# nlapier2/Metalign

Measured on AMD Instinct MI355X. Metric: 150bp reads/s end-to-end (CMash filter + profile), higher is better.
Workload: dtype u64; 1 GPU; configs[2]: 10M reads vs 10k-genome DB, multi-k {21,31,51} containment — 10000000 synthetic 150bp reads/GPU vs 10000-genome sketch DB (50000 bp genomes, n=1000), k in [21, 31, 51], 12498882 alignment records/GPU, 10001 taxa, 1 MI355X per rank; inputs resident in HBM; stage_a_definition=reference_pipeline, hash_mode=0, stage_a_match=kmer

## Files before the change

include/metalign_hip.h:

```cpp
#ifndef METALIGN_HIP_H
#define METALIGN_HIP_H

#include <stdint.h>

#ifdef __cplusplus
extern "C" {
#endif

#define MG_ABI_VERSION 1

typedef enum mg_status {
  MG_OK = 0,
  MG_ERR_HIP = -1,
  MG_ERR_ARG = -2,
  MG_ERR_CAPACITY = -3,
  MG_ERR_STATE = -4,
  MG_ERR_NOMEM = -5
} mg_status;

#define MG_MAX_K 64

typedef struct mg_aln_rec {
  uint32_t ref_new;
  uint32_t matched;
// ... 240 lines not shown
uint64_t mg_refdb_ngenomes(const mg_refdb* db);
uint64_t mg_refdb_max_hash(const mg_refdb* db);
const mg_db* mg_refdb_kmax_table(const mg_refdb* db);
void mg_refdb_free(mg_refdb* db);
int mg_refpipe_containment_dev(const mg_sketch* q, const mg_refdb* db, uint32_t ci, uint32_t* const* d_hits,
                               uint32_t* const* d_sizes);
int mg_refpipe_mark_dev(const mg_sketch* q, const mg_refdb* db, uint32_t ci, uint32_t* d_hits_kmax, uint32_t* d_sizes_kmax);
int mg_refpipe_count_dev(const mg_refdb* db, const uint32_t* const* d_marks, uint32_t* const* d_hits,
                         uint32_t* const* d_sizes);
int mg_refdb_marks(const mg_refdb* db, int ki, uint32_t** d_marks, uint64_t* nwords);

typedef struct mg_kcounts mg_kcounts;
int mg_refdb_index_kmers(mg_refdb* db, const uint64_t* kmer_hi, const uint64_t* kmer_lo);
int mg_refdb_has_kmer_index(const mg_refdb* db);
uint64_t mg_refdb_distinct_kmers(const mg_refdb* db);
int mg_refdb_kmer_heads(const mg_refdb* db, uint32_t* head);
int mg_kcounts_new(const mg_refdb* db, mg_kcounts** out);
int mg_kcounts_reset(mg_kcounts* kc);
int mg_count_kmers_dev(const uint8_t* d_bases, const uint64_t* d_offsets, uint64_t nreads, uint64_t nbases, const mg_refdb* db,
                       mg_kcounts* kc);
int mg_kcounts_stats(const mg_kcounts* kc, uint64_t* out4);
int mg_kcounts_download(const mg_kcounts* kc, const mg_refdb* db, uint32_t* per_pair);
int mg_kcounts_device(const mg_kcounts* kc, uint32_t** d_counts, uint64_t* n);
int mg_kcounts_wait(const mg_kcounts* kc);
uint64_t mg_kcounts_pack2_bytes(const mg_kcounts* kc);
int mg_kcounts_pack2_dev(const mg_kcounts* kc, uint32_t* d_out);
int mg_kcounts_merge2_dev(mg_kcounts* kc, const uint32_t* d_all, uint32_t nranks, uint64_t stride_dwords);
void mg_kcounts_free(mg_kcounts* kc);
int mg_refpipe_mark_counts_dev(const mg_kcounts* kc, const mg_refdb* db, uint32_t ci, uint32_t* d_hits_kmax, uint32_t* d_sizes_kmax);
int mg_refpipe_mark_counts_ptr_dev(const uint32_t* d_counts, const mg_refdb* db, uint32_t ci, uint32_t* d_hits_kmax,
                                   uint32_t* d_sizes_kmax);
int mg_refpipe_containment_counts_dev(const mg_kcounts* kc, const mg_refdb* db, uint32_t ci, uint32_t* const* d_hits,
                                      uint32_t* const* d_sizes);
int mg_refdb_set_count_share(const mg_refdb* db, uint32_t rank, uint32_t world);

typedef struct mg_profile mg_profile;

int mg_profile_begin_dev(const mg_aln_rec* d_recs, uint64_t nrecs,
                         int has_lookahead, const uint32_t* d_ref2tax,
                         uint32_t nref, uint32_t ntax, double pct_id,
                         mg_profile** out);
int mg_profile_acc_reset(uint64_t* d_count, uint64_t* d_bases, uint64_t* d_first_seen,
                         uint64_t* d_scalars, uint32_t ntax);
int mg_profile_map_launch(mg_profile* p);
int mg_profile_state_map(const mg_profile* p, uint8_t map[2]);
int mg_profile_map_words_dev(mg_profile* p, int64_t* d_out3);
// ... 158 lines not shown
```

metalign_amd/_hip.py:

```python
import ctypes
import os

import numpy as np

_HERE = os.path.dirname(os.path.abspath(__file__))
LIB_PATH = os.environ.get("MG_LIB_PATH") or os.path.join(_HERE, "libmetalign_hip.so")

REC_DTYPE = np.dtype([("ref_new", "<u4"), ("matched", "<u4"), ("total", "<u4"), ("flag_len", "<u4")])
NEW_BIT = 0x80000000
REF_MASK = 0x7FFFFFFF
LEN_SHIFT = 12
MAX_SEQLEN = (1 << 20) - 1
U64_MAX = 0xFFFFFFFFFFFFFFFF
MAX_K = 64

EXPORTS = [
    "mg_abi_version", "mg_debug_set", "mg_debug_get", "mg_device_count", "mg_init", "mg_init_on_stream", "mg_shutdown", "mg_last_error",
    "mg_device_name", "mg_mem_info", "mg_mem_trim", "mg_dev_malloc", "mg_dev_free", "mg_memcpy_h2d", "mg_memcpy_d2h", "mg_dev_memset", "mg_sync",
    "mg_host_alloc", "mg_host_free", "mg_memcpy_d2h_async", "mg_memcpy_h2d_async",
    "mg_event_create", "mg_event_record", "mg_event_synchronize", "mg_event_destroy", "mg_stage_c_side_stream", "mg_stage_a_side_stream", "mg_stage_a_workgroups_per_cu", "mg_stage_c_join",
    "mg_prof_enable", "mg_prof_only", "mg_prof_reset", "mg_prof_get",
    "mg_refdb_index_kmers", "mg_refdb_has_kmer_index", "mg_refdb_distinct_kmers", "mg_refdb_kmer_heads", "mg_kcounts_new", "mg_kcounts_reset", "mg_count_kmers_dev",
    "mg_kcounts_stats", "mg_kcounts_download", "mg_kcounts_device", "mg_kcounts_wait", "mg_kcounts_pack2_bytes", "mg_kcounts_pack2_dev", "mg_kcounts_merge2_dev", "mg_kcounts_free", "mg_refpipe_mark_counts_dev", "mg_refpipe_mark_counts_ptr_dev",
    "mg_refpipe_containment_counts_dev", "mg_refdb_set_count_share",
    "mg_set_count_saturation", "mg_count_saturation", "mg_set_hash_mode", "mg_hash_mode", "mg_hash_mode1_ks", "mg_sketch_reads_dev", "mg_sketch_reads_dev_async", "mg_sketch_reads_multi_dev_async", "mg_sketch_resolve", "mg_filter_build", "mg_filter_download", "mg_filter_from_bits", "mg_filter_log2_bits", "mg_filter_make_resident", "mg_filter_drop_resident", "mg_filter_use_resident", "mg_filter_resident_bytes", "mg_filter_free",
    "mg_sketch_reads_filtered_dev", "mg_sketch_reads_filtered_dev_async", "mg_sketch_from_pairs_dev", "mg_sketch_merge_dev", "mg_sketch_merge_dev_async", "mg_sketch_split", "mg_sketch_slice_words_dev", "mg_sketch_set_bound", "mg_sketch_size", "mg_sketch_truncated", "mg_sketch_last_hash",
    "mg_sketch_kmers_seen", "mg_sketch_device_ptrs", "mg_sketch_download", "mg_sketch_free", "mg_sketch_reads",
    "mg_sketch_stream_begin", "mg_sketch_stream_begin_counts", "mg_sketch_stream_add_dev", "mg_sketch_stream_add_file", "mg_sketch_stream_finish", "mg_sketch_stream_nreads", "mg_sketch_stream_nbases", "mg_sketch_stream_free",
    "mg_reads_parse_dev", "mg_reads_parse_prefix_dev", "mg_reads_parse", "mg_reads_parse_bam_prefix_dev", "mg_reads_from_bam_file", "mg_reads_count", "mg_reads_nbases", "mg_reads_device_ptrs",
    "mg_reads_download", "mg_reads_free",
    "mg_genomes_parse_dev", "mg_genomes_count", "mg_genomes_nbases", "mg_genomes_device_ptrs", "mg_genomes_download", "mg_genomes_free",
    "mg_genomes_stream_open", "mg_genomes_stream_next", "mg_genomes_stream_stats", "mg_genomes_stream_close",
    "mg_sketch_genomes_dev", "mg_sketch_genomes_prefix_dev", "mg_sketch_genomes_kmers_dev",
    "mg_acc_index_build", "mg_acc_index_free", "mg_sam_tokenize_dev", "mg_sam_tokenize", "mg_paf_tokenize_dev", "mg_paf_tokenize", "mg_sam_stream_file", "mg_bam_stream_file", "mg_bam_tokenize_dev", "mg_sam_batch_count",
    "mg_sam_batch_last_qname", "mg_sam_batch_device_ptr", "mg_sam_batch_download", "mg_sam_batch_free",
    "mg_sam_tokenize_keyed_dev", "mg_bam_tokenize_keyed_dev", "mg_sam_batch_keys_download", "mg_collate_order_dev", "mg_sam_batch_collate_dev",
    "mg_sam_stream_file_collated", "mg_bam_stream_file_collated",
    "mg_sam_tokenize_named_dev", "mg_sam_tokenize_named", "mg_bam_tokenize_named_dev", "mg_sam_stream_file_named", "mg_bam_stream_file_named",
    "mg_sam_batch_names_size", "mg_sam_batch_names_download", "mg_profile_commit_assign_dev",
    "mg_sam_tokenize_dev_ex", "mg_sam_tokenize_ex", "mg_bam_tokenize_dev_ex", "mg_sam_stream_file_ex", "mg_bam_stream_file_ex",
    "mg_sam_batch_places_download", "mg_sam_batch_places_device_ptr",
    "mg_coverage_create", "mg_coverage_add_dev", "mg_coverage_result", "mg_coverage_free",
    "mg_depth_create", "mg_depth_add_dev", "mg_depth_finish", "mg_depth_fetch_rows", "mg_depth_fetch_windows", "mg_depth_free",
    "mg_sam_batch_edits_download", "mg_sam_batch_edits_device_ptr",
    "mg_identity_create", "mg_identity_add_dev", "mg_identity_result", "mg_identity_fetch_hist", "mg_identity_free",
    "mg_sam_batch_bases_download", "mg_sam_batch_bases_device_ptr",
# ... 729 lines not shown
    def add_reads(self, reads):
        p_b, p_o = reads.device_ptrs()
        self.add_dev(p_b, p_o, reads.count, reads.nbases)

    def stats(self):
        out = np.zeros(12, np.uint64)
        self.hip._chk(self.hip.lib.mg_kcounts_stats(self.handle, _np(out, ctypes.c_uint64)))
        st = dict(kmers=int(out[0]), runs=int(out[1]), passed=int(out[2]), matches=int(out[3]))
        if out[6]:
            st.update(clk_drain=int(out[4]) * 64, clk_hits=int(out[5]) * 64, clk_kernel=int(out[6]) * 64, entries_looked_at=int(out[7]),
                      windows_scanned=int(out[8]), longest_lane_windows=int(out[9]), longest_lane_entries=int(out[10]), drains=int(out[11]))
        return st

    def download(self):
        npairs = self.table.sizes()[0]
        out = np.zeros(max(npairs, 1), np.uint32)
        self.hip._chk(self.hip.lib.mg_kcounts_download(self.handle, self.table.handle, _np(out, ctypes.c_uint32)))
        return out[:npairs]

    def device(self):
        p, n = _vp(), ctypes.c_uint64(0)
        self.hip._chk(self.hip.lib.mg_kcounts_device(self.handle, ctypes.byref(p), ctypes.byref(n)))
        return int(p.value or 0), int(n.value)

    def wait(self):
        self.hip._chk(self.hip.lib.mg_kcounts_wait(self.handle))

    def pack2_bytes(self):
        self.hip.lib.mg_kcounts_pack2_bytes.restype = ctypes.c_uint64
        return int(self.hip.lib.mg_kcounts_pack2_bytes(self.handle))

    def pack2_dev(self, d_out):
        self.hip._chk(self.hip.lib.mg_kcounts_pack2_dev(self.handle, ctypes.c_void_p(int(d_out))))

    def merge2_dev(self, d_all, nranks, stride_bytes):
        self.hip._chk(self.hip.lib.mg_kcounts_merge2_dev(self.handle, ctypes.c_void_p(int(d_all)), ctypes.c_uint32(int(nranks)),
                                                         ctypes.c_uint64(int(stride_bytes) // 4)))

    def free(self):
        if self.handle:
            self.hip.lib.mg_kcounts_free(self.handle)
            self.handle = None

    def __del__(self):
        try:
            self.free()
# ... 1316 lines not shown
```

metalign_amd/csrc/mg_contain.hip:

```cpp
#include <memory>

#include "mg_internal.h"

namespace mg {

constexpr int kMaxSmallK = 3;
struct ContainK {
  const uint64_t* q;
  const uint32_t* qc;
  uint64_t qn, q_last;
  const uint64_t* meta;
  uint32_t* idx;
  unsigned shift;
  uint64_t idx_buckets;
  uint32_t build_index;
  const uint64_t* ph;
  const uint32_t* pg;
  const uint32_t* gsize;
  uint64_t npairs, ngenomes;
  uint64_t tile0;
  uint32_t* hits_part;
  uint32_t* sizes_part;
  uint32_t* hits;
  uint32_t* sizes;
  const uint32_t* head;
// ... 290 lines not shown
      p[j] = 0xffffffffu; g[j] = 0;
      if (i < K.n) { p[j] = cid[i]; g[j] = cgen[i]; }
    }
    uint32_t w[kPer];
#pragma unroll
    for (int j = 0; j < kPer; ++j) w[j] = p[j] != 0xffffffffu ? marks[p[j] >> 5] : 0u;
#pragma unroll
    for (int j = 0; j < kPer; ++j)
      if ((w[j] >> (p[j] & 31u)) & 1u) atomicAdd(&hits[g[j]], 1u);
  }
}

__global__ void k_refpipe_reduce(const CountArgs a) {
  const uint64_t g0 = (uint64_t)blockIdx.x * blockDim.x + threadIdx.x;
  const uint64_t stride = (uint64_t)gridDim.x * blockDim.x;
  for (int ki = 0; ki < a.nk; ++ki) {
    const CountK& K = a.k[ki];
    for (uint64_t g = g0; g < K.ngenomes; g += stride) {
      uint32_t h = 0;
      for (uint32_t c = 0; c < a.copies; ++c) h += K.hits_part[(uint64_t)c * K.ngenomes + g];
      K.hits[g] = h;
      K.sizes[g] = K.gsize[g];
    }
  }
}

__global__ void k_iota_u32(uint32_t* v, uint64_t n) {
  uint64_t i = (uint64_t)blockIdx.x * blockDim.x + threadIdx.x;
  const uint64_t stride = (uint64_t)gridDim.x * blockDim.x;
  for (; i < n; i += stride) v[i] = (uint32_t)i;
}

__global__ void k_pair_genomes(const uint32_t* __restrict__ orig, uint64_t n, const uint64_t* __restrict__ offsets,
                               uint64_t ngenomes, uint32_t* __restrict__ pair_gen) {
  uint64_t i = (uint64_t)blockIdx.x * blockDim.x + threadIdx.x;
  const uint64_t stride = (uint64_t)gridDim.x * blockDim.x;
  for (; i < n; i += stride) {
    const uint64_t o = orig[i];
    uint64_t lo = 0, hi = ngenomes;
    while (hi - lo > 1) {
      const uint64_t mid = (lo + hi) >> 1;
      if (offsets[mid] <= o) lo = mid; else hi = mid;
    }
    pair_gen[i] = (uint32_t)lo;
  }
}
// ... 351 lines not shown
    K.cid = rp->small[s].cid.as<uint32_t>() + lo;
    K.cgen = rp->small[s].cgen.as<uint32_t>() + lo;
    K.n = hi - lo;
    K.tile0 = tiles;
    tiles += (K.n + kCTile - 1) / kCTile;
    K.ngenomes = G;
    K.marks = d_marks ? d_marks[s] : rp->marks.as<uint32_t>() + rp->small[s].marks_at;
    K.gsize = rp->small[s].gsize.as<uint32_t>();
    K.hits_part = d_part + (uint64_t)s * copies * G;
    K.hits = d_hits[s];
    K.sizes = d_sizes[s];
  }
  a.ntiles = tiles;
  ProfScope ps("refpipe_count");
  if (!prezeroed)
    hipLaunchKernelGGL(k_zero_u32, dim3(grid_for((uint64_t)m * copies * G, 256, (unsigned)c.num_cus * 8)), dim3(256), 0, st, d_part,
                       (uint64_t)m * copies * G);
  if (tiles) hipLaunchKernelGGL(k_refpipe_count, dim3(grid_cap(grid_for(tiles, 1, (unsigned)c.num_cus * 8), "kb_grid")), dim3(kCT), 0, st, a);
  hipLaunchKernelGGL(k_refpipe_reduce, dim3(grid_for(G, 256, (unsigned)c.num_cus * 4)), dim3(256), 0, st, a);
  MG_HIP(hipGetLastError());
  return MG_OK;
}

extern "C" {

int mg_containment_multi_dev(int nk, const mg_sketch* const* qs, const mg_db* const* dbs, uint32_t ci, uint32_t* const* d_hits,
                             uint32_t* const* d_sizes) {
  return containment_launch(nk, qs, dbs, ci, d_hits, d_sizes, nullptr);
}

int mg_refpipe_mark_dev(const mg_sketch* q, const mg_refdb* db, uint32_t ci, uint32_t* d_hits_kmax, uint32_t* d_sizes_kmax) {
  if (!q || !db) return fail(MG_ERR_ARG, "null argument");
  MG_TRY(refdb_ready(db));
  const mg_db* kdb = &db->kmax;
  return containment_launch(1, &q, &kdb, ci, &d_hits_kmax, &d_sizes_kmax, db);
}

int mg_refdb_set_count_share(const mg_refdb* db, uint32_t rank, uint32_t world) {
  if (!db || world == 0 || rank >= world) return fail(MG_ERR_ARG, "rank %u of %u", rank, world);
  db->share_rank = rank;
  db->share_world = world;
  return MG_OK;
}

int mg_refpipe_count_dev(const mg_refdb* db, const uint32_t* const* d_marks, uint32_t* const* d_hits, uint32_t* const* d_sizes) {
  MG_REQUIRE_READY();
// ... 13 lines not shown
  MG_REQUIRE_READY();
  if (!kc || !db || !d_hits_kmax || !d_sizes_kmax) return fail(MG_ERR_ARG, "null argument");
  MG_TRY(refdb_ready(db));
  if (!db->kidx) return fail(MG_ERR_STATE, "the table has no k-mer index (mg_refdb_index_kmers)");
  uint32_t* d_counts = nullptr;
  uint64_t n = 0;
  MG_TRY(mg_kcounts_device(kc, &d_counts, &n));
  if (n != db->kmax.total) return fail(MG_ERR_ARG, "these counters belong to another table");
  MG_TRY(kcounts_wait(kc));
  return match_launch(d_counts, db, ci, d_hits_kmax, d_sizes_kmax);
}

int mg_refpipe_mark_counts_ptr_dev(const uint32_t* d_counts, const mg_refdb* db, uint32_t ci, uint32_t* d_hits_kmax, uint32_t* d_sizes_kmax) {
  MG_REQUIRE_READY();
  if (!d_counts || !db || !d_hits_kmax || !d_sizes_kmax) return fail(MG_ERR_ARG, "null argument");
  MG_TRY(refdb_ready(db));
  if (!db->kidx) return fail(MG_ERR_STATE, "the table has no k-mer index (mg_refdb_index_kmers)");
  return match_launch(d_counts, db, ci, d_hits_kmax, d_sizes_kmax);
}

int mg_refpipe_containment_counts_dev(const mg_kcounts* kc, const mg_refdb* db, uint32_t ci, uint32_t* const* d_hits, uint32_t* const* d_sizes) {
  if (!kc || !db || !d_hits || !d_sizes) return fail(MG_ERR_ARG, "null argument");
  const int last = db->nk - 1;
  MG_TRY(mg_refpipe_mark_counts_dev(kc, db, ci, d_hits[last], d_sizes[last]));
  return refpipe_count_launch(db, nullptr, d_hits, d_sizes);
}

int mg_containment_dev(const mg_sketch* q, const mg_db* db, uint32_t ci, uint32_t* d_hits, uint32_t* d_sizes) {
  return mg_containment_multi_dev(1, &q, &db, ci, &d_hits, &d_sizes);
}

int mg_containment(const uint64_t* q_hashes, const uint32_t* q_counts, uint64_t qn, int q_truncated, uint32_t ci,
                   const uint64_t* db_hashes, const uint64_t* db_offsets, uint64_t ngenomes, uint32_t* out_hits,
                   uint32_t* out_sizes) {
  MG_REQUIRE_READY();
  std::unique_ptr<mg_sketch> sk(new mg_sketch());
  MG_TRY(sk->hashes.alloc(qn * sizeof(uint64_t)));
  MG_TRY(sk->counts.alloc(qn * sizeof(uint32_t)));
  MG_TRY(mg_memcpy_h2d(sk->hashes.p, q_hashes, qn * sizeof(uint64_t)));
  MG_TRY(mg_memcpy_h2d(sk->counts.p, q_counts, qn * sizeof(uint32_t)));
  sk->n = qn;
  sk->truncated = q_truncated;
  sk->last_hash = qn ? q_hashes[qn - 1] : 0;
  mg_db* db = nullptr;
  MG_TRY(mg_db_upload(db_hashes, db_offsets, ngenomes, &db));
  std::unique_ptr<mg_db> dbg(db);
// ... 11 lines not shown
```

metalign_amd/csrc/mg_core.hip:

```cpp
#include <cstring>

#include "mg_internal.h"

namespace mg {

static thread_local char g_err[512] = "";

Context& ctx() {
  static Context c;
  return c;
}

int fail(int code, const char* fmt, ...) {
  va_list ap;
  va_start(ap, fmt);
  vsnprintf(g_err, sizeof(g_err), fmt, ap);
  va_end(ap);
  return code;
}

static const char* const kDebugKeys[] = {
    "k3_hashed", "k3_flush_tiles", "k3_grid", "lds_pad", "force_list", "distinct_hint_ppm", "resident_scan", "no_fused", "resident_ablate",
    "flush_order", "no_avx2", "gzip_threads", "pgzip_chunk", "pgzip_thp", "pgzip_timing", "stream_thin", "stream_threads", "inflate_trace", "inflate_loose_find", "shares_threads", "kc_wg_per_cu", "kc_ablate", "kc_stagger", "kc_gate_extra", "inflate_dev_max_bytes", "kc_grid", "k1_grid", "kb_grid", "collate_defer", "genome_slab_bytes", "genome_guard", "cov_grid", "depth_grid", "mm_hash_bits", "ident_grid", "var_grid"};
static int64_t g_debug[sizeof(kDebugKeys) / sizeof(kDebugKeys[0])] = {};
static int debug_index(const char* key) {
  for (size_t i = 0; i < sizeof(kDebugKeys) / sizeof(kDebugKeys[0]); ++i)
    if (strcmp(kDebugKeys[i], key) == 0) return (int)i;
  return -1;
}
int64_t dbg(const char* key) {
  const int i = debug_index(key);
  return i < 0 ? 0 : g_debug[i];
}

static uint64_t size_class(uint64_t n) {
  if (n < 256) return 256;
  uint64_t p = 256;
  while (p < n) {
    if (p + p / 2 >= n) return p + p / 2;
    p <<= 1;
  }
  return p;
}

static void seal_open_batch();
static void release_completed_batches();
// ... 509 lines not shown
```

metalign_amd/csrc/mg_internal.h:

```cpp
#pragma once
#include <hip/hip_runtime.h>

#include <cstdarg>
#include <cstdlib>
#include <cstdint>
#include <cstdio>
#include <map>
#include <memory>
#include <string>
#include <utility>
#include <vector>

#include "../../include/metalign_hip.h"

namespace mg {

constexpr uint64_t kReservedHash = 0xFFFFFFFFFFFFFFFFull;

struct ProfEntry {
  uint64_t launches = 0;
  double total_ms = 0.0;
};

struct DevBuf;
// ... 321 lines not shown
struct mg_db {
  mg::DevBuf pair_hash;
  mg::DevBuf pair_gen;
  mg::DevBuf gsize;
  mg::DevBuf offsets;
  uint64_t ngenomes = 0;
  uint64_t total = 0;
  uint64_t max_hash = 0;
};

namespace mg {
struct KmerIndex {
  int k = 0;
  uint64_t ndistinct = 0, nentries = 0, nbuckets = 0;
  uint32_t gbits = 0;
  uint64_t gate_words = 0;
  uint32_t bmask = 0;
  DevBuf gate;
  DevBuf shared;
  DevBuf prim;
  DevBuf ovf;
  uint64_t novf = 0;
  DevBuf head;
};
int kcounts_wait(const mg_kcounts* kc);
}

struct mg_refdb {
  mg_db kmax;
  int nk = 0;
  int ks[4] = {0, 0, 0, 0};
  mg::DevBuf kmer_hi, kmer_lo;
  struct Small {
    mg::DevBuf pa, pb;
    mg::DevBuf cid, cgen;
    mg::DevBuf gsize;
    uint64_t nprefix = 0, ncount = 0;
    uint64_t marks_at = 0, marks_n = 0;
  } small[3];
  mg::DevBuf marks;
  uint64_t marks_words = 0;
  mutable uint32_t* count_part = nullptr;
  mutable uint32_t count_copies = 0;
  mutable uint64_t count_gen = 0;
  mutable mg::UploadJob* pending = nullptr;
  mutable bool unchecked = false;
  mutable uint32_t share_rank = 0, share_world = 1;
  mutable int failed = 0;
  std::unique_ptr<mg::KmerIndex> kidx;
  ~mg_refdb();
};
namespace mg { int refdb_ready(const mg_refdb* db); int check_pairs_dev(const mg_db& db); }
```

metalign_amd/csrc/mg_kcount.hip:

```cpp
#include <algorithm>
#include <memory>

#include "mg_internal.h"
#include "mg_kcount_core.h"
#include "mg_sketch_dev.h"

namespace mg {

namespace {

inline unsigned g256(uint64_t n) { return grid_for(n ? n : 1, 256, (unsigned)ctx().num_cus * 8); }
#define KC_FOR(i, n) for (uint64_t i = (uint64_t)blockIdx.x * blockDim.x + threadIdx.x; i < (n); i += (uint64_t)gridDim.x * blockDim.x)

__global__ void k_kc_canon(const uint64_t* __restrict__ khi, const uint64_t* __restrict__ klo, uint64_t n, int k,
                           uint64_t* __restrict__ chi, uint64_t* __restrict__ clo, uint32_t* __restrict__ iota) {
  KC_FOR(i, n) {
    const KcWin c = kc_canonical(kc_from_right(khi[i], klo[i], k), k);
    chi[i] = ((uint64_t)c.w[0] << 32) | c.w[1];
    clo[i] = ((uint64_t)c.w[2] << 32) | c.w[3];
    iota[i] = (uint32_t)i;
  }
}
__global__ void k_kc_gather(const uint64_t* __restrict__ src, const uint32_t* __restrict__ idx, uint64_t n, uint64_t* __restrict__ dst) {
  KC_FOR(i, n) dst[i] = src[idx[i]];
// ... 11 lines not shown
    const KcWin x{{(uint32_t)(hi[j] >> 32), (uint32_t)hi[j], (uint32_t)(lo[j] >> 32), (uint32_t)lo[j]}};
    dhi[id] = hi[j];
    dlo[id] = lo[j];
    dhead[id] = order[j];
    uint32_t keys[kKcMaxCands];
    nkeys[id] = (uint32_t)kc_table_keys(x, k, keys);
  }
}
__global__ void k_kc_emit_keys(const uint64_t* __restrict__ dhi, const uint64_t* __restrict__ dlo, const uint64_t* __restrict__ kbefore,
                               uint64_t nd, int k, uint32_t bmask, uint64_t* __restrict__ ekey, uint32_t* __restrict__ eid) {
  KC_FOR(id, nd) {
    const KcWin x{{(uint32_t)(dhi[id] >> 32), (uint32_t)dhi[id], (uint32_t)(dlo[id] >> 32), (uint32_t)dlo[id]}};
    uint32_t keys[kKcMaxCands];
    const int n = kc_table_keys(x, k, keys);
    for (int t = 0; t < n; ++t) {
      ekey[kbefore[id] + (uint64_t)t] = ((uint64_t)(keys[t] & bmask) << 32) | keys[t];
      eid[kbefore[id] + (uint64_t)t] = (uint32_t)id;
    }
  }
}
__global__ void k_kc_pair_heads(const uint32_t* __restrict__ order, const uint32_t* __restrict__ flag, const uint64_t* __restrict__ before,
                                const uint32_t* __restrict__ dhead, uint64_t n, uint32_t* __restrict__ head) {
  KC_FOR(j, n) head[order[j]] = dhead[before[j] + flag[j] - 1];
}
__global__ void k_kc_entries(const uint64_t* __restrict__ skey, const uint32_t* __restrict__ perm, const uint64_t* __restrict__ dhi,
                             const uint64_t* __restrict__ dlo, const uint32_t* __restrict__ dhead, uint64_t nd, int k, uint32_t gshift,
                             KcEntry* __restrict__ ent, uint32_t* __restrict__ gate, uint32_t* __restrict__ shared) {
  KC_FOR(j, nd) {
    const uint32_t id = perm[j];
    const uint64_t h = dhi[id], l = dlo[id];
    KcEntry e;
    e.w[0] = (uint32_t)(h >> 32); e.w[1] = (uint32_t)h; e.w[2] = (uint32_t)(l >> 32); e.w[3] = (uint32_t)l;
    e.head = dhead[id];
    e.key = (uint32_t)skey[j];
    e.off = kc_table_key_offset(KcWin{{e.w[0], e.w[1], e.w[2], e.w[3]}}, k, e.key);
    e.pad = 0;
    ent[j] = e;
    if (j == 0 || skey[j - 1] != skey[j]) {
      const uint32_t g = e.key >> gshift, bit = 1u << (g & 31u);
      if (atomicOr(&gate[g >> 5], bit) & bit) atomicOr(&shared[g >> 5], bit);
    }
  }
}
__global__ void k_kc_offsets(const uint64_t* __restrict__ skey, uint64_t nd, uint64_t nb, uint32_t* __restrict__ offs) {
  KC_FOR(j, nd + 1) {
    const uint64_t first = j == 0 ? 0 : (skey[j - 1] >> 32) + 1;
// ... 547 lines not shown
int kcounts_order(const mg_kcounts* kc, hipStream_t st) {
  if (kc && kc->ev && kc->ev_stream && kc->ev_stream != st) MG_HIP(hipStreamWaitEvent(st, kc->ev, 0));
  return MG_OK;
}
int kcounts_wait(const mg_kcounts* kc) { return kcounts_order(kc, ctx().stream); }
static int kcounts_wrote(mg_kcounts* kc, hipStream_t st) {
  MG_HIP(hipEventRecord(kc->ev, st));
  kc->ev_stream = st;
  return MG_OK;
}
static hipStream_t kcounts_stage_stream() {
  Context& c = ctx();
  return c.a_side ? (c.a_side == 2 ? c.stream_a2 : c.stream_a) : c.stream;
}

__global__ void k_kc_copy_words(const uint32_t* __restrict__ src, uint32_t* __restrict__ dst, uint64_t nwords) {
  const uint64_t n4 = nwords / 4;
  const uint4* __restrict__ s4 = reinterpret_cast<const uint4*>(src);
  uint4* __restrict__ d4 = reinterpret_cast<uint4*>(dst);
  KC_FOR(i, n4) d4[i] = s4[i];
  KC_FOR(i, nwords - 4 * n4) dst[4 * n4 + i] = src[4 * n4 + i];
}

__global__ void k_kc_pack2(const uint32_t* __restrict__ counts, uint64_t n, uint32_t* __restrict__ out) {
  KC_FOR(w, (n + 15) / 16) {
    uint32_t v = 0;
#pragma unroll
    for (int j = 0; j < 16; ++j) {
      const uint64_t i = w * 16 + (uint64_t)j;
      const uint32_t c = i < n ? counts[i] : 0u;
      v |= (c > 3u ? 3u : c) << (2 * j);
    }
    out[w] = v;
  }
}
__global__ void k_kc_merge2(const uint32_t* __restrict__ all, uint32_t nranks, uint64_t stride, uint64_t n, uint32_t* __restrict__ counts) {
  KC_FOR(w, (n + 15) / 16) {
    uint32_t s[16];
#pragma unroll
    for (int j = 0; j < 16; ++j) s[j] = 0;
    for (uint32_t r = 0; r < nranks; ++r) {
      const uint32_t v = all[(uint64_t)r * stride + w];
#pragma unroll
      for (int j = 0; j < 16; ++j) s[j] += (v >> (2 * j)) & 3u;
    }
#pragma unroll
// ... 31 lines not shown
  DevBuf chi, clo, iota, ord1, ord2, s_lo, s_hi, g_hi, flag, before, dhi, dlo, dhead, nkeys, kbefore, ekey, eid, skey, perm;
  uint64_t nd = 0, ne = 0;
  if (n) {
    MG_TRY(chi.alloc(n * 8)); MG_TRY(clo.alloc(n * 8)); MG_TRY(iota.alloc(n * 4)); MG_TRY(ord1.alloc(n * 4)); MG_TRY(ord2.alloc(n * 4));
    MG_TRY(s_lo.alloc(n * 8)); MG_TRY(s_hi.alloc(n * 8)); MG_TRY(g_hi.alloc(n * 8)); MG_TRY(flag.alloc(n * 4)); MG_TRY(before.alloc((n + 2) * 8));
    hipLaunchKernelGGL(k_kc_canon, dim3(g256(n)), dim3(256), 0, st, db->kmer_hi.as<uint64_t>(), db->kmer_lo.as<uint64_t>(), n, k,
                       chi.as<uint64_t>(), clo.as<uint64_t>(), iota.as<uint32_t>());
    MG_TRY(sort_pairs(clo.as<uint64_t>(), s_lo.as<uint64_t>(), iota.as<uint32_t>(), ord1.as<uint32_t>(), n));
    hipLaunchKernelGGL(k_kc_gather, dim3(g256(n)), dim3(256), 0, st, chi.as<uint64_t>(), ord1.as<uint32_t>(), n, g_hi.as<uint64_t>());
    MG_TRY(sort_pairs(g_hi.as<uint64_t>(), s_hi.as<uint64_t>(), ord1.as<uint32_t>(), ord2.as<uint32_t>(), n));
    hipLaunchKernelGGL(k_kc_gather, dim3(g256(n)), dim3(256), 0, st, clo.as<uint64_t>(), ord2.as<uint32_t>(), n, s_lo.as<uint64_t>());
    hipLaunchKernelGGL(k_kc_heads, dim3(g256(n)), dim3(256), 0, st, s_hi.as<uint64_t>(), s_lo.as<uint64_t>(), n, flag.as<uint32_t>());
    MG_HIP(hipGetLastError());
    MG_TRY(exclusive_sum_u32_to_u64(flag.as<uint32_t>(), before.as<uint64_t>(), n, &nd));
    MG_TRY(dhi.alloc(nd * 8)); MG_TRY(dlo.alloc(nd * 8)); MG_TRY(dhead.alloc(nd * 4)); MG_TRY(nkeys.alloc((nd + 1) * 4));
    MG_TRY(kbefore.alloc((nd + 2) * 8));
    hipLaunchKernelGGL(k_kc_distinct, dim3(g256(n)), dim3(256), 0, st, s_hi.as<uint64_t>(), s_lo.as<uint64_t>(), ord2.as<uint32_t>(),
                       flag.as<uint32_t>(), before.as<uint64_t>(), n, k, dhi.as<uint64_t>(), dlo.as<uint64_t>(), dhead.as<uint32_t>(),
                       nkeys.as<uint32_t>());
    hipLaunchKernelGGL(k_kc_pair_heads, dim3(g256(n)), dim3(256), 0, st, ord2.as<uint32_t>(), flag.as<uint32_t>(), before.as<uint64_t>(),
                       dhead.as<uint32_t>(), n, ix->head.as<uint32_t>());
    MG_HIP(hipGetLastError());
  }
  ix->ndistinct = nd;
  unsigned bb = 8;
  while (bb < 28 && (1ull << bb) < nd) ++bb;
  ix->bmask = (1u << bb) - 1u;
  ix->nbuckets = 1ull << bb;
  const int64_t gx = dbg("kc_gate_extra");
  ix->gbits = kc_gate_bits(nd, gx > 0 ? (uint32_t)gx : kKcGateExtra);
  ix->gate_words = (1ull << ix->gbits) / 32 + 2;
  MG_TRY(ix->gate.alloc(ix->gate_words * 4));
  MG_TRY(ix->shared.alloc(ix->gate_words * 4));
  MG_HIP(hipMemsetAsync(ix->gate.p, 0, ix->gate_words * 4, st));
  MG_HIP(hipMemsetAsync(ix->shared.p, 0, ix->gate_words * 4, st));
  if (nd) {
    MG_TRY(exclusive_sum_u32_to_u64(nkeys.as<uint32_t>(), kbefore.as<uint64_t>(), nd, &ne));
    MG_TRY(ekey.alloc((ne + 1) * 8)); MG_TRY(eid.alloc((ne + 1) * 4)); MG_TRY(skey.alloc((ne + 1) * 8)); MG_TRY(perm.alloc((ne + 1) * 4));
    hipLaunchKernelGGL(k_kc_emit_keys, dim3(g256(nd)), dim3(256), 0, st, dhi.as<uint64_t>(), dlo.as<uint64_t>(), kbefore.as<uint64_t>(), nd, k,
                       ix->bmask, ekey.as<uint64_t>(), eid.as<uint32_t>());
    MG_HIP(hipGetLastError());
    MG_TRY(sort_pairs(ekey.as<uint64_t>(), skey.as<uint64_t>(), eid.as<uint32_t>(), perm.as<uint32_t>(), ne));
  }
  ix->nentries = ne;
  DevBuf offs, ent, extra, obefore;
  MG_TRY(offs.alloc((ix->nbuckets + 2) * 4));
// ... 39 lines not shown
  if (!db->kidx) return fail(MG_ERR_STATE, "the table has no k-mer index (mg_refdb_index_kmers)");
  std::unique_ptr<mg_kcounts> kc(new mg_kcounts());
  kc->n = db->kmax.total;
  kc->live_words = db->kidx->gate_words;
  kc->sat_words = kKcSlots * db->kidx->nbuckets + db->kidx->novf + 4;
  kc->gate = db->kidx->gate.p;
  MG_TRY(kc->counts.alloc((kc->n + 1) * 4));
  MG_TRY(kc->live.alloc(kc->live_words * 4));
  MG_TRY(kc->sat.alloc(kc->sat_words * 4));
  MG_TRY(kc->stats.alloc(12 * 8));
  MG_HIP(hipEventCreateWithFlags(&kc->ev, hipEventDisableTiming));
  MG_TRY(mg_kcounts_reset(kc.get()));
  *out = kc.release();
  return MG_OK;
}

int mg_kcounts_reset(mg_kcounts* kc) {
  MG_REQUIRE_READY();
  if (!kc) return fail(MG_ERR_ARG, "null argument");
  Context& c = ctx();
  if (!c.stream_r) MG_HIP(hipStreamCreateWithFlags(&c.stream_r, hipStreamNonBlocking));
  hipStream_t st = c.stream_r;
  MG_TRY(kcounts_order(kc, st));
  hipLaunchKernelGGL(k_kc_copy_words, dim3(g256(kc->live_words / 4 + 1)), dim3(256), 0, st, static_cast<const uint32_t*>(kc->gate),
                     kc->live.as<uint32_t>(), kc->live_words);
  MG_HIP(hipGetLastError());
  kc->epoch = kc->epoch % 255u + 1u;
  if (kc->epoch == 1u) MG_HIP(hipMemsetAsync(kc->sat.p, 0, kc->sat_words * 4, st));
  MG_HIP(hipMemsetAsync(kc->counts.p, 0, (kc->n + 1) * 4, st));
  MG_HIP(hipMemsetAsync(kc->stats.p, 0, 12 * 8, st));
  return kcounts_wrote(kc, st);
}

int mg_kcounts_wait(const mg_kcounts* kc) {
  MG_REQUIRE_READY();
  if (!kc) return fail(MG_ERR_ARG, "null argument");
  return kcounts_wait(kc);
}

uint64_t mg_kcounts_pack2_bytes(const mg_kcounts* kc) { return kc ? ((kc->n + 15) / 16) * 4 : 0; }

int mg_kcounts_pack2_dev(const mg_kcounts* kc, uint32_t* d_out) {
  MG_REQUIRE_READY();
  if (!kc || !d_out) return fail(MG_ERR_ARG, "null argument");
  if (ctx().count_sat == 0 || ctx().count_sat > 3)
    return fail(MG_ERR_STATE, "two bits hold a counter that saturates at 3 or below (it saturates at %u): exchange the counters themselves", ctx().count_sat);
  MG_TRY(kcounts_wait(kc));
  if (kc->n) hipLaunchKernelGGL(k_kc_pack2, dim3(g256((kc->n + 15) / 16)), dim3(256), 0, ctx().stream, kc->counts.as<uint32_t>(), kc->n, d_out);
  MG_HIP(hipGetLastError());
  return MG_OK;
}

int mg_kcounts_merge2_dev(mg_kcounts* kc, const uint32_t* d_all, uint32_t nranks, uint64_t stride_dwords) {
// ... 56 lines not shown
}

int mg_kcounts_download(const mg_kcounts* kc, const mg_refdb* db, uint32_t* per_pair) {
  MG_REQUIRE_READY();
  if (!kc || !db || !db->kidx || !per_pair) return fail(MG_ERR_ARG, "null argument");
  if (kc->n != db->kmax.total) return fail(MG_ERR_ARG, "these counters belong to another table");
  if (!kc->n) return MG_OK;
  MG_TRY(kcounts_wait(kc));
  DevBuf out;
  MG_TRY(out.alloc(kc->n * 4));
  hipLaunchKernelGGL(k_kc_per_pair, dim3(g256(kc->n)), dim3(256), 0, ctx().stream, kc->counts.as<uint32_t>(), db->kidx->head.as<uint32_t>(),
                     kc->n, ctx().count_sat, out.as<uint32_t>());
  MG_HIP(hipGetLastError());
  return mg_memcpy_d2h(per_pair, out.p, kc->n * 4);
}

int mg_kcounts_device(const mg_kcounts* kc, uint32_t** d_counts, uint64_t* n) {
  if (!kc || !d_counts || !n) return fail(MG_ERR_ARG, "null argument");
  *d_counts = kc->counts.as<uint32_t>();
  *n = kc->n;
  return MG_OK;
}

void mg_kcounts_free(mg_kcounts* kc) { delete kc; }

}
```

Measured before the change: 4.748 billion reads/s.

## Add sparse containment path walking only qualifying k-mer chains, fuse count reset

Adds a sparse containment path. It compacts k-mer pairs whose counts pass the threshold into LDS, follows per-distinct-kmer chains via a new `next` array, and marks and counts smaller-k prefix runs through per-prefix offset tables. Hits go into replicated per-genome copies that a separate kernel reduces, which replaces the dense mark+count pass over all pairs. Counter reset now runs as one fused kernel instead of a copy plus two memsets. The new path costs extra index memory, a one-time offset build, and chain-walking divergence; it falls back to the dense path when not applicable.

```diff
diff --git a/include/metalign_hip.h b/include/metalign_hip.h
--- a/include/metalign_hip.h
+++ b/include/metalign_hip.h
@@ -286,6 +286,7 @@
 int mg_kcounts_stats(const mg_kcounts* kc, uint64_t* out4);
 int mg_kcounts_download(const mg_kcounts* kc, const mg_refdb* db, uint32_t* per_pair);
 int mg_kcounts_device(const mg_kcounts* kc, uint32_t** d_counts, uint64_t* n);
+int mg_kcounts_gate_dev(const mg_kcounts* kc, uint32_t** d_live, const uint32_t** d_gate, uint64_t* words);
 int mg_kcounts_wait(const mg_kcounts* kc);
 uint64_t mg_kcounts_pack2_bytes(const mg_kcounts* kc);
 int mg_kcounts_pack2_dev(const mg_kcounts* kc, uint32_t* d_out);
diff --git a/metalign_amd/_hip.py b/metalign_amd/_hip.py
--- a/metalign_amd/_hip.py
+++ b/metalign_amd/_hip.py
@@ -21,7 +21,7 @@
     "mg_event_create", "mg_event_record", "mg_event_synchronize", "mg_event_destroy", "mg_stage_c_side_stream", "mg_stage_a_side_stream", "mg_stage_a_workgroups_per_cu", "mg_stage_c_join",
     "mg_prof_enable", "mg_prof_only", "mg_prof_reset", "mg_prof_get",
     "mg_refdb_index_kmers", "mg_refdb_has_kmer_index", "mg_refdb_distinct_kmers", "mg_refdb_kmer_heads", "mg_kcounts_new", "mg_kcounts_reset", "mg_count_kmers_dev",
-    "mg_kcounts_stats", "mg_kcounts_download", "mg_kcounts_device", "mg_kcounts_wait", "mg_kcounts_pack2_bytes", "mg_kcounts_pack2_dev", "mg_kcounts_merge2_dev", "mg_kcounts_free", "mg_refpipe_mark_counts_dev", "mg_refpipe_mark_counts_ptr_dev",
+    "mg_kcounts_stats", "mg_kcounts_download", "mg_kcounts_device", "mg_kcounts_gate_dev", "mg_kcounts_wait", "mg_kcounts_pack2_bytes", "mg_kcounts_pack2_dev", "mg_kcounts_merge2_dev", "mg_kcounts_free", "mg_refpipe_mark_counts_dev", "mg_refpipe_mark_counts_ptr_dev",
     "mg_refpipe_containment_counts_dev", "mg_refdb_set_count_share",
     "mg_set_count_saturation", "mg_count_saturation", "mg_set_hash_mode", "mg_hash_mode", "mg_hash_mode1_ks", "mg_sketch_reads_dev", "mg_sketch_reads_dev_async", "mg_sketch_reads_multi_dev_async", "mg_sketch_resolve", "mg_filter_build", "mg_filter_download", "mg_filter_from_bits", "mg_filter_log2_bits", "mg_filter_make_resident", "mg_filter_drop_resident", "mg_filter_use_resident", "mg_filter_resident_bytes", "mg_filter_free",
     "mg_sketch_reads_filtered_dev", "mg_sketch_reads_filtered_dev_async", "mg_sketch_from_pairs_dev", "mg_sketch_merge_dev", "mg_sketch_merge_dev_async", "mg_sketch_split", "mg_sketch_slice_words_dev", "mg_sketch_set_bound", "mg_sketch_size", "mg_sketch_truncated", "mg_sketch_last_hash",
@@ -797,6 +797,11 @@
         p, n = _vp(), ctypes.c_uint64(0)
         self.hip._chk(self.hip.lib.mg_kcounts_device(self.handle, ctypes.byref(p), ctypes.byref(n)))
         return int(p.value or 0), int(n.value)
+
+    def gate(self):
+        live, gate, n = _vp(), _vp(), ctypes.c_uint64(0)
+        self.hip._chk(self.hip.lib.mg_kcounts_gate_dev(self.handle, ctypes.byref(live), ctypes.byref(gate), ctypes.byref(n)))
+        return int(live.value or 0), int(gate.value or 0), int(n.value)
 
     def wait(self):
         self.hip._chk(self.hip.lib.mg_kcounts_wait(self.handle))
diff --git a/metalign_amd/csrc/mg_contain.hip b/metalign_amd/csrc/mg_contain.hip
--- a/metalign_amd/csrc/mg_contain.hip
+++ b/metalign_amd/csrc/mg_contain.hip
@@ -1,6 +1,7 @@
 #include <memory>
 
 #include "mg_internal.h"
+#include "mg_match_core.h"
 
 namespace mg {
 
@@ -337,6 +338,152 @@
       K.hits[g] = h;
       K.sizes[g] = K.gsize[g];
     }
+  }
+}
+
+struct SparseArgs {
+  const uint32_t* counts;
+  MsView v;
+  uint64_t ngenomes;
+  uint32_t ci, cs, copies;
+  const uint32_t* gsize[kMaxContainK];
+  uint32_t* out_hits[kMaxContainK];
+  uint32_t* out_sizes[kMaxContainK];
+};
+constexpr int kMsPer = 8;
+constexpr int kMsTile = kMsPer * kCT;
+
+__device__ __forceinline__ void ms_wave_runs(const MsView& v, const MsRuns& r, uint32_t lane) {
+#pragma unroll
+  for (int s = 0; s < kMsMaxSmall; ++s) {
+    if (s >= v.nsmall) break;
+#pragma unroll
+    for (int t = 0; t < 2; ++t) {
+      unsigned long long m = __ballot(r.b[2 * s + t] != r.a[2 * s + t]);
+      while (m) {
+        const int l = __builtin_ctzll(m);
+        m &= m - 1ull;
+        const uint32_t a = (uint32_t)__builtin_amdgcn_readlane((int)r.a[2 * s + t], l);
+        const uint32_t b = (uint32_t)__builtin_amdgcn_readlane((int)r.b[2 * s + t], l);
+        ms_run_part(v.cgen[s], v.hits[s], a, b, lane, kMsLanes);
+      }
+    }
+  }
+}
+
+__device__ __forceinline__ void ms_wave_heads(const MsView& v, bool have, uint32_t h, uint32_t lane) {
+  uint32_t i = have ? h : kMsNone;
+  for (uint32_t step = 0; step < kMsChainInline; ++step) {
+    if (__ballot(i != kMsNone) == 0ull) break;
+    MsRuns r;
+    uint32_t nx;
+    ms_pair(v, i != kMsNone, i, h, r, nx);
+    ms_wave_runs(v, r, lane);
+    i = nx;
+  }
+  unsigned long long m = __ballot(i != kMsNone);
+  while (m) {
+    const int l = __builtin_ctzll(m);
+    m &= m - 1ull;
+    const uint32_t H = (uint32_t)__builtin_amdgcn_readlane((int)h, l);
+    uint32_t I = (uint32_t)__builtin_amdgcn_readlane((int)i, l);
+    while (I != kMsNone) {
+      const uint64_t idx = (uint64_t)I + lane;
+      MsRuns r;
+      uint32_t nx;
+      const bool mem = ms_pair(v, idx < v.npairs, (uint32_t)idx, H, r, nx);
+      ms_wave_runs(v, r, lane);
+      const unsigned long long mm = __ballot(mem);
+      if (mm == 0ull) break;
+      I = (uint32_t)__builtin_amdgcn_readlane((int)nx, 63 - (int)__builtin_clzll(mm));
+    }
+  }
+}
+
+__global__ __launch_bounds__(kCT) void k_match_sparse(const SparseArgs a) {
+  __shared__ uint32_t s_q[kMsTile];
+  __shared__ uint32_t s_n;
+  const uint32_t tid = threadIdx.x, lane = tid & 63u, wave = tid >> 6;
+  MsView v = a.v;
+  {
+    const uint64_t copy = (uint64_t)(blockIdx.x & (a.copies - 1)) * a.ngenomes;
+    v.hits_kmax += copy;
+#pragma unroll
+    for (int s = 0; s < kMsMaxSmall; ++s)
+      if (s < v.nsmall) v.hits[s] += copy;
+  }
+  const uint32_t* __restrict__ counts = a.counts;
+  const uint64_t n = v.npairs, ntiles = (n + kMsTile - 1) / kMsTile;
+  const unsigned long long below = (1ull << lane) - 1ull;
+  uint32_t c[kMsPer];
+  auto load_tile = [&](uint64_t tile) {
+    const uint64_t t0 = tile * kMsTile;
+#pragma unroll
+    for (int j = 0; j < kMsPer / 4; ++j) {
+      const uint64_t i4 = t0 + 4ull * (tid + (uint32_t)kCT * j);
+      if (tile < ntiles && i4 + 4 <= n) {
+        const uint4 x = reinterpret_cast<const uint4*>(counts)[i4 >> 2];
+        c[4 * j] = x.x; c[4 * j + 1] = x.y; c[4 * j + 2] = x.z; c[4 * j + 3] = x.w;
+      } else {
+#pragma unroll
+        for (int u = 0; u < 4; ++u) c[4 * j + u] = (tile < ntiles && i4 + u < n) ? counts[i4 + u] : 0u;
+      }
+    }
+  };
+  load_tile(blockIdx.x);
+  for (uint64_t tile = blockIdx.x; tile < ntiles; tile += gridDim.x) {
+    if (tid == 0) s_n = 0;
+    __syncthreads();
+    const uint64_t t0 = tile * kMsTile;
+    uint32_t qm = 0, tot = 0;
+#pragma unroll
+    for (int j = 0; j < kMsPer; ++j) {
+      const bool q = ms_qualifies(c[j], a.ci, a.cs);
+      qm |= q ? 1u << j : 0u;
+      tot += (uint32_t)__popcll(__ballot(q));
+    }
+    uint32_t at = 0;
+    if (lane == 0 && tot) at = atomicAdd(&s_n, tot);
+    at = (uint32_t)__builtin_amdgcn_readfirstlane((int)at);
+#pragma unroll
+    for (int j = 0; j < kMsPer; ++j) {
+      const bool q = (qm >> j) & 1u;
+      const unsigned long long m = __ballot(q);
+      if (q) s_q[at + (uint32_t)__popcll(m & below)] = (uint32_t)(t0 + 4ull * (tid + (uint32_t)kCT * (j >> 2)) + (uint32_t)(j & 3));
+      at += (uint32_t)__popcll(m);
+    }
+    load_tile(tile + gridDim.x);
+    __syncthreads();
+    const uint32_t nq = s_n;
+    const uint32_t per = nq < (uint32_t)kCT ? (nq + 3u) / 4u : 64u;
+    for (uint32_t c0 = wave * per; c0 < nq && v.ablate != 1u; c0 += 4u * per) {
+      const bool have = lane < per && c0 + lane < nq;
+      ms_wave_heads(v, have, have ? s_q[c0 + lane] : 0u, lane);
+    }
+    __syncthreads();
+  }
+}
+
+__global__ void k_sparse_reduce(const SparseArgs a) {
+  const uint64_t g0 = (uint64_t)blockIdx.x * blockDim.x + threadIdx.x;
+  const uint64_t stride = (uint64_t)gridDim.x * blockDim.x;
+  for (int ki = 0; ki <= a.v.nsmall; ++ki) {
+    const uint32_t* __restrict__ part = ki < a.v.nsmall ? a.v.hits[ki] : a.v.hits_kmax;
+    for (uint64_t g = g0; g < a.ngenomes; g += stride) {
+      uint32_t h = 0;
+      for (uint32_t c = 0; c < a.copies; ++c) h += part[(uint64_t)c * a.ngenomes + g];
+      a.out_hits[ki][g] = h;
+      a.out_sizes[ki][g] = a.gsize[ki][g];
+    }
+  }
+}
+
+__global__ void k_count_offsets(const uint32_t* __restrict__ cid, uint64_t ncount, uint64_t nprefix, uint32_t* __restrict__ coff) {
+  const uint64_t stride = (uint64_t)gridDim.x * blockDim.x;
+  for (uint64_t j = (uint64_t)blockIdx.x * blockDim.x + threadIdx.x; j <= ncount; j += stride) {
+    const uint64_t first = j == 0 ? 0 : (uint64_t)cid[j - 1] + 1;
+    const uint64_t last = j == ncount ? nprefix : cid[j];
+    for (uint64_t p = first; p <= last; ++p) coff[p] = (uint32_t)j;
   }
 }
 
@@ -734,6 +881,90 @@
   return MG_OK;
 }
 
+static bool sparse_wanted(const mg_refdb* rp) {
+  return !dbg("kb_dense") && rp->share_world == 1 && rp->kidx && rp->kidx->next.p && rp->coff_state >= 0;
+}
+static bool sparse_ready(const mg_refdb* rp) {
+  if (!sparse_wanted(rp)) return false;
+  if (rp->coff_state > 0) return true;
+  Context& c = ctx();
+  const int m = rp->nk - 1;
+  bool ok = dbg("kb_sparse_alloc_fail") != 2;
+  for (int s = 0; s < m; ++s) ok = ok && rp->small[s].ncount < 0xfffffff0ull && rp->small[s].nprefix < 0xfffffff0ull;
+  ProfScope ps("contain_index");
+  for (int s = 0; s < m && ok; ++s) ok = rp->small[s].coff.alloc((rp->small[s].nprefix + 2) * sizeof(uint32_t)) == MG_OK;
+  for (int s = 0; s < m && ok; ++s) {
+    const mg_refdb::Small& S = rp->small[s];
+    hipLaunchKernelGGL(k_count_offsets, dim3(grid_for(S.ncount + 1, 256, (unsigned)c.num_cus * 8)), dim3(256), 0, c.stream,
+                       S.cid.as<uint32_t>(), S.ncount, S.nprefix, S.coff.as<uint32_t>());
+    ok = hipGetLastError() == hipSuccess;
+  }
+  if (!ok)
+    for (int s = 0; s < m; ++s) rp->small[s].coff.release();
+  rp->coff_state = ok ? 1 : -1;
+  return ok;
+}
+
+static int sparse_launch(const uint32_t* d_counts, const mg_refdb* rp, uint32_t ci, uint32_t* const* d_hits, uint32_t* const* d_sizes) {
+  Context& c = ctx();
+  hipStream_t st = c.stream;
+  if (c.count_sat && ci > c.count_sat)
+    return fail(MG_ERR_ARG, "count threshold ci=%u above the counters' saturation cs=%u: nothing could ever match", ci, c.count_sat);
+  const mg_db* db = &rp->kmax;
+  if (db->ngenomes == 0) return MG_OK;
+  if (ci == 0) return fail(MG_ERR_ARG, "ci = 0 would match every pair");
+  const int m = rp->nk - 1;
+  const uint64_t G = db->ngenomes;
+  SparseArgs a{};
+  a.counts = d_counts;
+  a.ngenomes = G;
+  a.ci = ci;
+  a.cs = c.count_sat;
+  uint32_t copies = 1;
+  for (; copies < 64 && 2ull * copies * G <= 65536; copies *= 2) {}
+  a.copies = copies;
+  const uint64_t part_total = (uint64_t)(m + 1) * copies * G;
+  uint32_t* d_part = (uint32_t*)scratch("contain_part", part_total * sizeof(uint32_t));
+  if (!d_part) return MG_ERR_NOMEM;
+  ++g_contain_gen;
+  MsView& v = a.v;
+  v.head = rp->kidx->head.as<uint32_t>();
+  v.next = rp->kidx->next.as<uint32_t>();
+  v.pg = db->pair_gen.as<uint32_t>();
+  v.npairs = db->total;
+  v.nsmall = m;
+  v.ablate = (uint32_t)dbg("kb_sparse_ablate");
+  v.hits_kmax = d_part + (uint64_t)m * copies * G;
+  a.gsize[m] = db->gsize.as<uint32_t>();
+  a.out_hits[m] = d_hits[m];
+  a.out_sizes[m] = d_sizes[m];
+  for (int s = 0; s < m; ++s) {
+    const mg_refdb::Small& S = rp->small[s];
+    v.pa[s] = S.pa.as<uint32_t>();
+    v.pb[s] = S.pb.as<uint32_t>();
+    v.coff[s] = S.coff.as<uint32_t>();
+    v.cgen[s] = S.cgen.as<uint32_t>();
+    v.marks[s] = rp->marks.as<uint32_t>() + S.marks_at;
+    v.hits[s] = d_part + (uint64_t)s * copies * G;
+    a.gsize[s] = S.gsize.as<uint32_t>();
+    a.out_hits[s] = d_hits[s];
+    a.out_sizes[s] = d_sizes[s];
+  }
+  ContainArgs z{};
+  z.zero = d_part;
+  z.nzero = part_total;
+  z.zero2 = rp->marks.as<uint32_t>();
+  z.nzero2 = rp->marks_words;
+  const uint64_t ntiles = (v.npairs + kMsTile - 1) / kMsTile;
+  ProfScope ps("containment");
+  const uint64_t work = z.nzero > z.nzero2 ? z.nzero : z.nzero2;
+  hipLaunchKernelGGL(k_build_index, dim3(grid_for(work ? work : 1, 256, (unsigned)c.num_cus * 16)), dim3(256), 0, st, z);
+  if (ntiles) hipLaunchKernelGGL(k_match_sparse, dim3(grid_cap(grid_for(ntiles, 1, (unsigned)c.num_cus * 8), "kb_grid")), dim3(kCT), 0, st, a);
+  hipLaunchKernelGGL(k_sparse_reduce, dim3(grid_for(G, 256, (unsigned)c.num_cus * 4)), dim3(256), 0, st, a);
+  MG_HIP(hipGetLastError());
+  return MG_OK;
+}
+
 extern "C" {
 
 int mg_containment_multi_dev(int nk, const mg_sketch* const* qs, const mg_db* const* dbs, uint32_t ci, uint32_t* const* d_hits,
@@ -793,6 +1024,23 @@
 int mg_refpipe_containment_counts_dev(const mg_kcounts* kc, const mg_refdb* db, uint32_t ci, uint32_t* const* d_hits, uint32_t* const* d_sizes) {
   if (!kc || !db || !d_hits || !d_sizes) return fail(MG_ERR_ARG, "null argument");
   const int last = db->nk - 1;
+  MG_REQUIRE_READY();
+  MG_TRY(refdb_ready(db));
+  if (sparse_wanted(db)) {
+    for (int ki = 0; ki <= last; ++ki)
+      if (!d_hits[ki] || !d_sizes[ki]) return fail(MG_ERR_ARG, "null argument");
+    uint32_t* d_counts = nullptr;
+    uint64_t n = 0;
+    MG_TRY(mg_kcounts_device(kc, &d_counts, &n));
+    if (n != db->kmax.total) return fail(MG_ERR_ARG, "these counters belong to another table");
+    if (ctx().count_sat && ci > ctx().count_sat)
+      return fail(MG_ERR_ARG, "count threshold ci=%u above the counters' saturation cs=%u: nothing could ever match", ci, ctx().count_sat);
+    if (ci == 0 && db->kmax.ngenomes) return fail(MG_ERR_ARG, "ci = 0 would match every pair");
+    if (sparse_ready(db)) {
+      MG_TRY(kcounts_wait(kc));
+      return sparse_launch(d_counts, db, ci, d_hits, d_sizes);
+    }
+  }
   MG_TRY(mg_refpipe_mark_counts_dev(kc, db, ci, d_hits[last], d_sizes[last]));
   return refpipe_count_launch(db, nullptr, d_hits, d_sizes);
 }
diff --git a/metalign_amd/csrc/mg_core.hip b/metalign_amd/csrc/mg_core.hip
--- a/metalign_amd/csrc/mg_core.hip
+++ b/metalign_amd/csrc/mg_core.hip
@@ -21,7 +21,7 @@
 
 static const char* const kDebugKeys[] = {
     "k3_hashed", "k3_flush_tiles", "k3_grid", "lds_pad", "force_list", "distinct_hint_ppm", "resident_scan", "no_fused", "resident_ablate",
-    "flush_order", "no_avx2", "gzip_threads", "pgzip_chunk", "pgzip_thp", "pgzip_timing", "stream_thin", "stream_threads", "inflate_trace", "inflate_loose_find", "shares_threads", "kc_wg_per_cu", "kc_ablate", "kc_stagger", "kc_gate_extra", "inflate_dev_max_bytes", "kc_grid", "k1_grid", "kb_grid", "collate_defer", "genome_slab_bytes", "genome_guard", "cov_grid", "depth_grid", "mm_hash_bits", "ident_grid", "var_grid"};
+    "flush_order", "no_avx2", "gzip_threads", "pgzip_chunk", "pgzip_thp", "pgzip_timing", "stream_thin", "stream_threads", "inflate_trace", "inflate_loose_find", "shares_threads", "kc_wg_per_cu", "kc_ablate", "kc_stagger", "kc_gate_extra", "inflate_dev_max_bytes", "kc_grid", "k1_grid", "kb_grid", "collate_defer", "genome_slab_bytes", "genome_guard", "cov_grid", "depth_grid", "mm_hash_bits", "ident_grid", "var_grid", "kb_dense", "kb_sparse_alloc_fail", "kb_sparse_ablate"};
 static int64_t g_debug[sizeof(kDebugKeys) / sizeof(kDebugKeys[0])] = {};
 static int debug_index(const char* key) {
   for (size_t i = 0; i < sizeof(kDebugKeys) / sizeof(kDebugKeys[0]); ++i)
diff --git a/metalign_amd/csrc/mg_internal.h b/metalign_amd/csrc/mg_internal.h
--- a/metalign_amd/csrc/mg_internal.h
+++ b/metalign_amd/csrc/mg_internal.h
@@ -367,6 +367,7 @@
   DevBuf ovf;
   uint64_t novf = 0;
   DevBuf head;
+  DevBuf next;
 };
 int kcounts_wait(const mg_kcounts* kc);
 }
@@ -382,6 +383,7 @@
     mg::DevBuf gsize;
     uint64_t nprefix = 0, ncount = 0;
     uint64_t marks_at = 0, marks_n = 0;
+    mutable mg::DevBuf coff;
   } small[3];
   mg::DevBuf marks;
   uint64_t marks_words = 0;
@@ -391,6 +393,7 @@
   mutable mg::UploadJob* pending = nullptr;
   mutable bool unchecked = false;
   mutable uint32_t share_rank = 0, share_world = 1;
+  mutable int coff_state = 0;
   mutable int failed = 0;
   std::unique_ptr<mg::KmerIndex> kidx;
   ~mg_refdb();
diff --git a/metalign_amd/csrc/mg_kcount.hip b/metalign_amd/csrc/mg_kcount.hip
--- a/metalign_amd/csrc/mg_kcount.hip
+++ b/metalign_amd/csrc/mg_kcount.hip
@@ -57,6 +57,9 @@
 __global__ void k_kc_pair_heads(const uint32_t* __restrict__ order, const uint32_t* __restrict__ flag, const uint64_t* __restrict__ before,
                                 const uint32_t* __restrict__ dhead, uint64_t n, uint32_t* __restrict__ head) {
   KC_FOR(j, n) head[order[j]] = dhead[before[j] + flag[j] - 1];
+}
+__global__ void k_kc_chain(const uint32_t* __restrict__ order, const uint32_t* __restrict__ flag, uint64_t n, uint32_t* __restrict__ next) {
+  KC_FOR(j, n) next[order[j]] = (j + 1 < n && !flag[j + 1]) ? order[j + 1] : 0xffffffffu;
 }
 __global__ void k_kc_entries(const uint64_t* __restrict__ skey, const uint32_t* __restrict__ perm, const uint64_t* __restrict__ dhi,
                              const uint64_t* __restrict__ dlo, const uint32_t* __restrict__ dhead, uint64_t nd, int k, uint32_t gshift,
@@ -650,6 +653,20 @@
   KC_FOR(i, nwords - 4 * n4) dst[4 * n4 + i] = src[4 * n4 + i];
 }
 
+__global__ __launch_bounds__(256) void k_kc_reset(const uint32_t* __restrict__ gate, uint32_t* __restrict__ live, uint64_t live_words,
+                                                  uint32_t* __restrict__ counts, uint64_t ncounts, uint32_t* __restrict__ stats,
+                                                  uint32_t nstats) {
+  const uint64_t l4 = live_words / 4, c4 = ncounts / 4;
+  const uint4* __restrict__ s4 = reinterpret_cast<const uint4*>(gate);
+  uint4* __restrict__ d4 = reinterpret_cast<uint4*>(live);
+  uint4* __restrict__ z4 = reinterpret_cast<uint4*>(counts);
+  KC_FOR(i, l4) d4[i] = s4[i];
+  KC_FOR(i, c4) z4[i] = make_uint4(0u, 0u, 0u, 0u);
+  KC_FOR(i, live_words - 4 * l4) live[4 * l4 + i] = gate[4 * l4 + i];
+  KC_FOR(i, ncounts - 4 * c4) counts[4 * c4 + i] = 0u;
+  KC_FOR(i, nstats) stats[i] = 0u;
+}
+
 __global__ void k_kc_pack2(const uint32_t* __restrict__ counts, uint64_t n, uint32_t* __restrict__ out) {
   KC_FOR(w, (n + 15) / 16) {
     uint32_t v = 0;
@@ -727,6 +744,10 @@
                        dhead.as<uint32_t>(), n, ix->head.as<uint32_t>());
     MG_HIP(hipGetLastError());
   }
+  if (dbg("kb_sparse_alloc_fail") != 1 && ix->next.alloc((n + 1) * 4) == MG_OK) {
+    if (n) hipLaunchKernelGGL(k_kc_chain, dim3(g256(n)), dim3(256), 0, st, ord2.as<uint32_t>(), flag.as<uint32_t>(), n, ix->next.as<uint32_t>());
+    MG_HIP(hipGetLastError());
+  }
   ix->ndistinct = nd;
   unsigned bb = 8;
   while (bb < 28 && (1ull << bb) < nd) ++bb;
@@ -812,13 +833,12 @@
   if (!c.stream_r) MG_HIP(hipStreamCreateWithFlags(&c.stream_r, hipStreamNonBlocking));
   hipStream_t st = c.stream_r;
   MG_TRY(kcounts_order(kc, st));
-  hipLaunchKernelGGL(k_kc_copy_words, dim3(g256(kc->live_words / 4 + 1)), dim3(256), 0, st, static_cast<const uint32_t*>(kc->gate),
-                     kc->live.as<uint32_t>(), kc->live_words);
+  const uint64_t most = std::max(kc->live_words, kc->n + 1) / 4 + 1;
+  hipLaunchKernelGGL(k_kc_reset, dim3(g256(most)), dim3(256), 0, st, static_cast<const uint32_t*>(kc->gate), kc->live.as<uint32_t>(),
+                     kc->live_words, kc->counts.as<uint32_t>(), kc->n + 1, kc->stats.as<uint32_t>(), 2u * 12u);
   MG_HIP(hipGetLastError());
   kc->epoch = kc->epoch % 255u + 1u;
   if (kc->epoch == 1u) MG_HIP(hipMemsetAsync(kc->sat.p, 0, kc->sat_words * 4, st));
-  MG_HIP(hipMemsetAsync(kc->counts.p, 0, (kc->n + 1) * 4, st));
-  MG_HIP(hipMemsetAsync(kc->stats.p, 0, 12 * 8, st));
   return kcounts_wrote(kc, st);
 }
 
@@ -921,6 +941,14 @@
   return MG_OK;
 }
 
+int mg_kcounts_gate_dev(const mg_kcounts* kc, uint32_t** d_live, const uint32_t** d_gate, uint64_t* words) {
+  if (!kc || !d_live || !d_gate || !words) return fail(MG_ERR_ARG, "null argument");
+  *d_live = kc->live.as<uint32_t>();
+  *d_gate = static_cast<const uint32_t*>(kc->gate);
+  *words = kc->live_words;
+  return MG_OK;
+}
+
 void mg_kcounts_free(mg_kcounts* kc) { delete kc; }
 
 }
diff --git a/metalign_amd/csrc/mg_match_core.h b/metalign_amd/csrc/mg_match_core.h
--- /dev/null
+++ b/metalign_amd/csrc/mg_match_core.h
@@ -0,0 +1,97 @@
+#pragma once
+#include <cstdint>
+
+#ifdef MG_HOST_CHECK
+#define MS_HD static inline
+#define MS_ADD1(ptr) (void)(++*(ptr))
+#define MS_OR(ptr, v) ms_host_or((ptr), (v))
+static inline uint32_t ms_host_or(uint32_t* p, uint32_t v) { const uint32_t old = *p; *p = old | v; return old; }
+#else
+#include <hip/hip_runtime.h>
+#define MS_HD __device__ __forceinline__
+#define MS_ADD1(ptr) (void)atomicAdd((ptr), 1u)
+#define MS_OR(ptr, v) atomicOr((ptr), (v))
+#endif
+
+namespace mg {
+
+constexpr int kMsMaxSmall = 3;
+constexpr uint32_t kMsNone = 0xffffffffu;
+constexpr uint32_t kMsRunInline = 16;
+constexpr uint32_t kMsChainInline = 8;
+constexpr uint32_t kMsLanes = 64;
+
+struct MsView {
+  const uint32_t* head;
+  const uint32_t* next;
+  const uint32_t* pg;
+  uint64_t npairs;
+  uint32_t* hits_kmax;
+  int nsmall;
+  uint32_t ablate;
+  const uint32_t* pa[kMsMaxSmall];
+  const uint32_t* pb[kMsMaxSmall];
+  const uint32_t* coff[kMsMaxSmall];
+  const uint32_t* cgen[kMsMaxSmall];
+  uint32_t* marks[kMsMaxSmall];
+  uint32_t* hits[kMsMaxSmall];
+};
+
+struct MsRuns {
+  uint32_t a[2 * kMsMaxSmall], b[2 * kMsMaxSmall];
+};
+
+MS_HD bool ms_qualifies(uint32_t c, uint32_t ci, uint32_t cs) {
+  const uint32_t v = (cs && c > cs) ? cs : c;
+  return v >= ci;
+}
+
+MS_HD void ms_run_part(const uint32_t* cgen, uint32_t* hits, uint32_t a, uint32_t b, uint32_t lane, uint32_t nlanes) {
+  for (uint64_t e = (uint64_t)a + lane; e < b; e += nlanes) MS_ADD1(&hits[cgen[e]]);
+}
+
+MS_HD bool ms_pair(const MsView& v, bool there, uint32_t i, uint32_t h, MsRuns& r, uint32_t& next) {
+  constexpr int kN = 2 * kMsMaxSmall;
+  uint32_t p[kN], old[kN], g0[kN];
+  const bool active = there && v.head[i] == h;
+  next = kMsNone;
+  uint32_t gk = 0;
+  if (active) { next = v.next[i]; gk = v.pg[i]; }
+#pragma unroll
+  for (int s = 0; s < kMsMaxSmall; ++s) {
+    p[2 * s] = p[2 * s + 1] = kMsNone;
+    if (s < v.nsmall && active && v.ablate != 2u) {
+      p[2 * s] = v.pa[s][i];
+      p[2 * s + 1] = v.pb[s][i];
+    }
+  }
+  if (active) MS_ADD1(&v.hits_kmax[gk]);
+#pragma unroll
+  for (int s = 0; s < kMsMaxSmall; ++s)
+    if (p[2 * s + 1] == p[2 * s]) p[2 * s + 1] = kMsNone;
+#pragma unroll
+  for (int j = 0; j < kN; ++j) {
+    old[j] = 0xffffffffu;
+    if (p[j] != kMsNone) old[j] = MS_OR(&v.marks[j >> 1][p[j] >> 5], 1u << (p[j] & 31u));
+  }
+#pragma unroll
+  for (int j = 0; j < kN; ++j) {
+    r.a[j] = r.b[j] = 0;
+    if (p[j] != kMsNone && !((old[j] >> (p[j] & 31u)) & 1u) && v.ablate != 3u) { r.a[j] = v.coff[j >> 1][p[j]]; r.b[j] = v.coff[j >> 1][p[j] + 1u]; }
+  }
+#pragma unroll
+  for (int j = 0; j < kN; ++j) {
+    g0[j] = 0;
+    if (r.b[j] != r.a[j] && r.b[j] - r.a[j] <= kMsRunInline) g0[j] = v.cgen[j >> 1][r.a[j]];
+  }
+#pragma unroll
+  for (int j = 0; j < kN; ++j) {
+    if (r.b[j] == r.a[j] || r.b[j] - r.a[j] > kMsRunInline) continue;
+    MS_ADD1(&v.hits[j >> 1][g0[j]]);
+    ms_run_part(v.cgen[j >> 1], v.hits[j >> 1], r.a[j] + 1u, r.b[j], 0u, 1u);
+    r.a[j] = r.b[j] = 0;
+  }
+  return active;
+}
+
+}
```

After: 4.821 billion reads/s, median of 6. Within noise of the previous version (+1.5%).
